# faris-k/self-supervised-wafermaps

Hardware: AMD Instinct MI355X
Metric: imgs/sec (SimCLR ResNet18, bs=256, 224^2) (higher is better)
Workload: dtype bf16; 1 GPU; SimCLR ResNet-18, 256 wafers/GPU/step, two 3x224x224 views, NT-Xent in-batch negatives, SGD (BASELINE.json configs[1]); per_gpu_batch=256, global_batch=256, parallelism=dp1, hip_graph=True, backward_stage_graphs=1, parallel_branches=two views through the backbone

## Files before the change

self-supervised-wafermaps_amd/csrc/bn.hip:

```cpp
#include "common.h"

namespace {

constexpr int BN_THREADS = 256;

__device__ __forceinline__ void unpack8(const uint4 v, float (&f)[8]) {
  f[0] = bf2f((uint16_t)(v.x & 0xffff)); f[1] = bf2f((uint16_t)(v.x >> 16));
  f[2] = bf2f((uint16_t)(v.y & 0xffff)); f[3] = bf2f((uint16_t)(v.y >> 16));
  f[4] = bf2f((uint16_t)(v.z & 0xffff)); f[5] = bf2f((uint16_t)(v.z >> 16));
  f[6] = bf2f((uint16_t)(v.w & 0xffff)); f[7] = bf2f((uint16_t)(v.w >> 16));
}
__device__ __forceinline__ uint4 pack8(const float (&f)[8]) {
  return make_uint4(pack_bf2(f[0], f[1]), pack_bf2(f[2], f[3]), pack_bf2(f[4], f[5]), pack_bf2(f[6], f[7]));
}

struct PoolSrc {
  const uint16_t* dy;
  const uint8_t* idx;
  int H, W, P, Q;
};

__device__ __forceinline__ void pool_grad8(const PoolSrc& ps, uint32_t row, int C, int c0, float (&g)[8]) {
  const uint32_t hw = (uint32_t)(ps.H * ps.W);
  const int n = (int)(row / hw);
// ... 373 lines not shown
        coef[((size_t)g * 7 + 1) * C + c] = is;
        coef[((size_t)g * 7 + 2) * C + c] = sc;
        coef[((size_t)g * 7 + 3) * C + c] = (float)(s1 / rows_per_group);
        coef[((size_t)g * 7 + 4) * C + c] = (float)(s2 / rows_per_group);
        coef[((size_t)g * 7 + 5) * C + c] = sc;
        coef[((size_t)g * 7 + 6) * C + c] = (beta ? beta[c] : 0.f) - mu * sc;
      }
    }
  }
  if (owner) {
    if (dgamma) dgamma[c] = (accumulate ? dgamma[c] : 0.f) + (float)tg;
    if (dbeta) dbeta[c] = (accumulate ? dbeta[c] : 0.f) + (float)tb;
  }
}

template <bool POW2, int FORM>
__global__ __launch_bounds__(BN_THREADS, FORM == 0 ? 4 : 1) void bn_bwd_apply(const uint16_t* __restrict__ y,
                                                           const uint16_t* __restrict__ dout,
                                                           const uint16_t* __restrict__ out,
                                                           const float* __restrict__ coef,
                                                           long long rows, int C, int rows_per_group,
                                                           int remask, int cshift, uint16_t* __restrict__ dy,
                                                           uint16_t* __restrict__ dz, const PoolSrc ps) {
  const int cpr = C >> 3;
  const long long total = rows * cpr;
  int cur_g = -1;
  constexpr int NK = FORM == 0 ? 5 : 7;
  float k[NK][8];
  for (long long p = (long long)blockIdx.x * BN_THREADS + threadIdx.x; p < total;
       p += (long long)gridDim.x * BN_THREADS) {
    long long row;
    int c0, g;
    if (POW2) {
      row = p >> cshift;
      c0 = (int)(p & (cpr - 1)) * 8;
      g = 0;
      for (long long lim = rows_per_group; row >= lim; lim += rows_per_group) ++g;
    } else {
      row = p / cpr;
      c0 = (int)(p - row * cpr) * 8;
      g = (int)(row / rows_per_group);
    }
    if (!POW2 || g != cur_g) {
      const float* cf = coef + (size_t)g * 7 * C + c0;
#pragma unroll
      for (int t = 0; t < NK; ++t) {
        const float4 a = *reinterpret_cast<const float4*>(cf + (size_t)t * C);
        const float4 b = *reinterpret_cast<const float4*>(cf + (size_t)t * C + 4);
        k[t][0] = a.x; k[t][1] = a.y; k[t][2] = a.z; k[t][3] = a.w;
        k[t][4] = b.x; k[t][5] = b.y; k[t][6] = b.z; k[t][7] = b.w;
      }
      cur_g = g;
    }
    const size_t off = row * C + c0;
    float fy[8], fd[8];
    unpack8(*reinterpret_cast<const uint4*>(y + off), fy);
    if constexpr (FORM == 2) pool_grad8(ps, (uint32_t)row, C, c0, fd);
    else unpack8(*reinterpret_cast<const uint4*>(dout + off), fd);
    if constexpr (FORM != 0) {
      if (out) {
        float fo[8];
        unpack8(*reinterpret_cast<const uint4*>(out + off), fo);
#pragma unroll
        for (int e = 0; e < 8; ++e) fd[e] = fo[e] > 0.f ? fd[e] : 0.f;
      }
      if (!out && remask) {
#pragma unroll
        for (int e = 0; e < 8; ++e) fd[e] = bf2f(f2bf(fmaf(fy[e], k[NK - 2][e], k[NK - 1][e]))) > 0.f ? fd[e] : 0.f;
      }
      if (dz) *reinterpret_cast<uint4*>(dz + off) = pack8(fd);
    }
    float r[8];
#pragma unroll
    for (int e = 0; e < 8; ++e) {
      const float xh = (fy[e] - k[0][e]) * k[1][e];
      r[e] = k[2][e] * (fd[e] - k[3][e] - xh * k[4][e]);
    }
    *reinterpret_cast<uint4*>(dy + off) = pack8(r);
  }
}

__global__ __launch_bounds__(BN_THREADS) void bn_pool_bwd_apply(const uint16_t* __restrict__ y,
                                                                const float* __restrict__ coef, int n_coef, int N, int C,
                                                                int imgs_per_group, int remask,
                                                                uint16_t* __restrict__ dy, const PoolSrc ps,
                                                                const WmDiv d_cpr, const WmDiv d_wb, const WmDiv d_ha,
                                                                const WmDiv d_ipg) {
  const uint32_t cpr = (uint32_t)C >> 3;
  const uint32_t HA = (uint32_t)ps.H >> 1, WB = (uint32_t)ps.W >> 1;
  const uint32_t total = (uint32_t)N * HA * WB * cpr;
  extern __shared__ __attribute__((aligned(16))) float pool_coef[];
  for (int i = threadIdx.x; i < n_coef; i += BN_THREADS) pool_coef[i] = coef[i];
  __syncthreads();
  for (uint32_t t = blockIdx.x * BN_THREADS + threadIdx.x; t < total; t += gridDim.x * BN_THREADS) {
    uint32_t rc, rb, ra;
    uint32_t u = wm_divmod(t, d_cpr, rc);
    const int c0 = (int)rc * 8;
    u = wm_divmod(u, d_wb, rb);
    const int n = (int)wm_divmod(u, d_ha, ra);
    const int b = (int)rb, a = (int)ra;
    const int g = (int)wm_div((uint32_t)n, d_ipg);
    const float* kk = pool_coef + (size_t)g * 7 * C + c0;
    auto krow = [&](int q, float (&v)[8]) {
      const float4 lo = *reinterpret_cast<const float4*>(kk + q * C);
      const float4 hi = *reinterpret_cast<const float4*>(kk + q * C + 4);
      v[0] = lo.x; v[1] = lo.y; v[2] = lo.z; v[3] = lo.w; v[4] = hi.x; v[5] = hi.y; v[6] = hi.z; v[7] = hi.w;
    };
    uint2 pk[4];
    uint4 dv[4];
    bool wok[4];
#pragma unroll
    for (int j = 0; j < 4; ++j) {
      const int p = a + (j >> 1), q = b + (j & 1);
      wok[j] = p < ps.P && q < ps.Q;
      const int pc = p < ps.P ? p : ps.P - 1, qc = q < ps.Q ? q : ps.Q - 1;
      const size_t o = ((size_t)(n * ps.P + pc) * ps.Q + qc) * C + c0;
      pk[j] = *reinterpret_cast<const uint2*>(ps.idx + o);
      dv[j] = *reinterpret_cast<const uint4*>(ps.dy + o);
    }
    float dw[4][8];
#pragma unroll
    for (int j = 0; j < 4; ++j) unpack8(dv[j], dw[j]);
#pragma unroll
    for (int pix = 0; pix < 4; ++pix) {
      const int dh = pix >> 1, dwp = pix & 1;
      float fd[8];
#pragma unroll
      for (int e = 0; e < 8; ++e) fd[e] = 0.f;
#pragma unroll
      for (int j = 0; j < 4; ++j) {
        const int kh = dh + 1 - 2 * (j >> 1), kw = dwp + 1 - 2 * (j & 1);
        if (kh < 0 || kw < 0) continue;
        const int code = kh * 3 + kw;
        if (wok[j]) {
#pragma unroll
          for (int e = 0; e < 8; ++e) {
            const int ie = (int)(((e < 4 ? pk[j].x : pk[j].y) >> (8 * (e & 3))) & 0xff);
            fd[e] += ie == code ? dw[j][e] : 0.f;
          }
        }
      }
#pragma unroll
      for (int e = 0; e < 8; ++e) fd[e] = bf2f(f2bf(fd[e]));
      const size_t off = ((size_t)(n * ps.H + 2 * a + dh) * ps.W + 2 * b + dwp) * C + c0;
      float fy[8];
      unpack8(*reinterpret_cast<const uint4*>(y + off), fy);
      if (remask) {
        float k5[8], k6[8];
        krow(5, k5);
        krow(6, k6);
#pragma unroll
        for (int e = 0; e < 8; ++e) fd[e] = bf2f(f2bf(fmaf(fy[e], k5[e], k6[e]))) > 0.f ? fd[e] : 0.f;
      }
      float r[8], k0[8], k1[8];
      krow(0, k0);
      krow(1, k1);
#pragma unroll
      for (int e = 0; e < 8; ++e) r[e] = (fy[e] - k0[e]) * k1[e];
      krow(4, k0);
      krow(3, k1);
#pragma unroll
      for (int e = 0; e < 8; ++e) r[e] = fd[e] - k1[e] - r[e] * k0[e];
      krow(2, k0);
#pragma unroll
      for (int e = 0; e < 8; ++e) r[e] = k0[e] * r[e];
      *reinterpret_cast<uint4*>(dy + off) = pack8(r);
    }
  }
}

__global__ __launch_bounds__(BN_THREADS) void stats_prereduce(const float* __restrict__ in, int T, int R, int To, int GC2,
                                                              int C2, float* __restrict__ out) {
  const long long i = (long long)blockIdx.x * BN_THREADS + threadIdx.x;
  const long long total = (long long)GC2 / C2 * To * C2;
  if (i >= total) return;
  const int c2 = (int)(i % C2);
  const long long u = i / C2;
  const int to = (int)(u % To), g = (int)(u / To);
  const float* src = in + ((size_t)g * T + (size_t)to * R) * C2 + c2;
  const int n = min(R, T - to * R);
  float v = 0.f;
  int k = 0;
  for (; k + 8 <= n; k += 8) {
    float t[8];
#pragma unroll
    for (int q = 0; q < 8; ++q) t[q] = src[(size_t)(k + q) * C2];
#pragma unroll
    for (int q = 0; q < 8; ++q) v += t[q];
  }
  for (; k < n; ++k) v += src[(size_t)k * C2];
  out[i] = v;
}

constexpr int STAT_SLOTS_DIRECT = 512, STAT_SLOTS_REDUCED = 128;
inline size_t stat_scratch_floats(int T, int G, int C) {
  return T > STAT_SLOTS_DIRECT ? (size_t)G * STAT_SLOTS_REDUCED * 2 * C : 0;
}

inline const float* stat_partials(const float* stat_part, int T, int G, int C, float* scratch, int* nblk, hipStream_t st) {
  if (T <= STAT_SLOTS_DIRECT) {
    *nblk = T;
    return stat_part;
  }
  int R = 1;
  while ((T + R - 1) / R > STAT_SLOTS_REDUCED) R *= 2;
  const int To = (T + R - 1) / R;
  const long long total = (long long)G * To * 2 * C;
  stats_prereduce<<<wm_cdiv(total, BN_THREADS), BN_THREADS, 0, st>>>(stat_part, T, R, To, G * 2 * C, 2 * C, scratch);
  *nblk = To;
  return scratch;
}

inline bool chunk_pow2(int C, int* shift) {
  const int cpr = C >> 3;
  if (cpr <= 0 || (cpr & (cpr - 1)) || BN_THREADS % cpr) return false;
  int sft = 0;
  while ((1 << sft) < cpr) ++sft;
  *shift = sft;
  return true;
}

__global__ __launch_bounds__(BN_THREADS) void add_bf16_kernel(const uint16_t* __restrict__ a,
                                                              const uint16_t* __restrict__ b,
                                                              long long n8, uint16_t* __restrict__ o) {
  for (long long p = (long long)blockIdx.x * BN_THREADS + threadIdx.x; p < n8;
       p += (long long)gridDim.x * BN_THREADS) {
    float fa[8], fb[8];
    unpack8(reinterpret_cast<const uint4*>(a)[p], fa);
    unpack8(reinterpret_cast<const uint4*>(b)[p], fb);
#pragma unroll
    for (int e = 0; e < 8; ++e) fa[e] += fb[e];
    reinterpret_cast<uint4*>(o)[p] = pack8(fa);
  }
}

inline int reduce_blocks(int rows_per_group, int C) {
  const int tpr = C >> 3;
  const int rpp = BN_THREADS / tpr > 0 ? BN_THREADS / tpr : 1;
  int nblk = wm_cdiv(rows_per_group, rpp * 16);
  if (nblk > 256) nblk = 256;
  if (nblk < 1) nblk = 1;
  return nblk;
}

inline int stream_grid(long long items) {
  long long b = (items + BN_THREADS - 1) / BN_THREADS;
  if (b > 256 * 16) b = 256 * 16;
  if (b < 1) b = 1;
  return (int)b;
// ... 206 lines not shown
  launch_finalize(bn_fwd_finalize, C, st, part, nblk, G, C, rpg, 0, gamma, beta, eps, momentum, running_mean, running_var,
                  num_batches_tracked, save_mean, save_invstd, scale, shift);
  WM_LAUNCH_CHECK();
  return WM_OK;
}

int bn_train_fwd_impl(const void* y_, const void* residual, const float* gamma, const float* beta, float* running_mean,
                      float* running_var, long long* num_batches_tracked, long long rows, int C, int G, float eps,
                      float momentum, int relu, float* save_mean, float* save_invstd, void* out_, void* relu_mask,
                      const float* stat_part, int stat_tiles, void* workspace, size_t workspace_bytes, void* stream) {
  WM_REQUIRE(y_ && out_ && save_mean && save_invstd && workspace, WM_EINVAL);
  const int rc = bn_shape_check(rows, C, G);
  if (rc != WM_OK) return rc;
  const size_t need = stat_part ? ((size_t)2 * G * C + stat_scratch_floats(stat_tiles, G, C)) * sizeof(float)
                                : wm_bn_workspace_bytes(rows, C, G);
  WM_REQUIRE(workspace_bytes >= need, WM_EWORKSPACE);
  hipStream_t st = static_cast<hipStream_t>(stream);
  const uint16_t *y = bf16(y_), *res = bf16(residual);
  uint16_t* out = bf16(out_);
  const int rpg = (int)(rows / G);
  if (!stat_part && bn_wide(rows, C, G)) {
    WM_REQUIRE(relu_mask == nullptr, WM_EUNSUPPORTED);
    bn_col_fwd<<<wm_cdiv(C, BN_THREADS), BN_THREADS, 0, st>>>(y, res, gamma, beta, running_mean, running_var,
                                                              num_batches_tracked, rpg, C, G, eps, momentum, relu, 1,
                                                              save_mean, save_invstd, out);
    WM_LAUNCH_CHECK();
    return WM_OK;
  }
  float* scale = static_cast<float*>(workspace);
  float* shift = scale + (size_t)G * C;
  const int rs = bn_fwd_stats(y, stat_part, stat_tiles, gamma, beta, running_mean, running_var, num_batches_tracked, rpg, C, G,
                              eps, momentum, save_mean, save_invstd, scale, shift, shift + (size_t)G * C, st);
  if (rs != WM_OK) return rs;
  launch_bn_apply(y, res, scale, shift, rows, C, rpg, relu, out, st, static_cast<uint8_t*>(relu_mask));
  WM_LAUNCH_CHECK();
  return WM_OK;
}

int bn_bwd_impl(const void* y_, const void* dout_, const void* out_relu_, int relu_from_y, const float* gamma,
                const float* beta, const float* save_mean, const float* save_invstd, long long rows, int C, int G,
                float* dgamma, float* dbeta, int accumulate, void* dy_, void* dz_, void* workspace, size_t workspace_bytes,
                void* stream, const PoolSrc ps, const void* ysel) {
  WM_REQUIRE(y_ && (dout_ || ps.dy) && save_mean && save_invstd && dy_ && workspace, WM_EINVAL);
  const int rc = bn_shape_check(rows, C, G);
  if (rc != WM_OK) return rc;
  WM_REQUIRE(workspace_bytes >= wm_bn_workspace_bytes(rows, C, G), WM_EWORKSPACE);
  hipStream_t st = static_cast<hipStream_t>(stream);
  const uint16_t *y = bf16(y_), *dout = bf16(dout_), *out_relu = bf16(out_relu_);
  uint16_t *dy = bf16(dy_), *dz = bf16(dz_);
  const int rpg = (int)(rows / G);
  const bool remask = relu_remask(relu_from_y, out_relu);
  if (bn_wide(rows, C, G)) {
    WM_REQUIRE(ps.dy == nullptr && dout, WM_EUNSUPPORTED);
    bn_col_bwd<<<wm_cdiv(C, BN_THREADS), BN_THREADS, 0, st>>>(y, dout, out_relu, remask ? 1 : 0, gamma, beta, save_mean,
                                                              save_invstd, rpg, C, G, dgamma, dbeta, accumulate, dy, dz);
    WM_LAUNCH_CHECK();
    return WM_OK;
  }
  const int nblk = reduce_blocks(rpg, C);
  float* part = static_cast<float*>(workspace);
  float* coef = part + (size_t)G * nblk * 2 * C;
  const int tpr = C >> 3;
  WM_REQUIRE(!remask || (gamma && beta), WM_EINVAL);
  int nblk_used = nblk;
  if (ps.dy != nullptr && ysel != nullptr) {
    const long long prow = (long long)(rows / ((long long)ps.H * ps.W)) * ps.P * ps.Q;
    WM_REQUIRE(prow % G == 0, WM_EUNSUPPORTED);
    const int prpg = (int)(prow / G);
    nblk_used = reduce_blocks(prpg, C);
    if (nblk_used > nblk) nblk_used = nblk;
    launch_reduce<1>(bf16(ysel), ps.dy, nullptr, save_mean, save_invstd, gamma, beta, prpg, C, G, nblk_used, part, PoolSrc{},
                     st);
  } else {
    launch_reduce<1>(y, dout, out_relu, save_mean, save_invstd, remask ? gamma : nullptr, remask ? beta : nullptr, rpg, C, G,
                     nblk, part, ps, st);
  }
  WM_LAUNCH_CHECK();
  launch_finalize(bn_bwd_finalize, C, st, part, nblk_used, G, C, rpg, gamma, beta, save_mean, save_invstd, dgamma, dbeta,
                  accumulate, coef, 0);
  WM_LAUNCH_CHECK();
  if (ps.dy != nullptr && !dz && !out_relu && (ps.H & 1) == 0 && (ps.W & 1) == 0 && BN_THREADS % tpr == 0 &&
      rows * tpr < (1ll << 31) && (size_t)G * 7 * C * sizeof(float) <= 32768) {
    const int n_img = (int)(rows / ((long long)ps.H * ps.W));
    bn_pool_bwd_apply<<<stream_grid(rows / 4 * tpr), BN_THREADS, (size_t)G * 7 * C * sizeof(float), st>>>(
        y, coef, G * 7 * C, n_img, C, n_img / G, remask ? 1 : 0, dy, ps, wm_div_make((uint32_t)(C >> 3)),
        wm_div_make((uint32_t)(ps.W >> 1)), wm_div_make((uint32_t)(ps.H >> 1)), wm_div_make((uint32_t)(n_img / G)));
    WM_LAUNCH_CHECK();
    return WM_OK;
  }
  const int form = ps.dy != nullptr ? 2 : (out_relu == nullptr && !remask && dz == nullptr) ? 0 : 1;
  launch_bn_bwd_apply(form, y, dout, out_relu, coef, rows, C, rpg, remask, dy, dz, ps, st);
  WM_LAUNCH_CHECK();
  return WM_OK;
}

}

extern "C" size_t wm_bn_workspace_bytes(long long rows, int C, int G) {
  if (rows <= 0 || C <= 0 || G <= 0 || C % 8) return 0;
  const int nblk = reduce_blocks((int)(rows / G), C);
  return ((size_t)G * nblk * 2 * C + (size_t)G * 7 * C) * sizeof(float) + 256;
}

extern "C" int wm_bn_train_fwd(const void* y, const void* residual, const float* gamma,
                               const float* beta, float* running_mean, float* running_var,
                               long long* num_batches_tracked, long long rows, int C, int G, float eps, float momentum, int relu,
                               float* save_mean, float* save_invstd, void* out, void* relu_mask, void* workspace,
                               size_t workspace_bytes, void* stream) {
  return bn_train_fwd_impl(y, residual, gamma, beta, running_mean, running_var, num_batches_tracked, rows, C, G, eps, momentum,
                           relu, save_mean, save_invstd, out, relu_mask, nullptr, 0, workspace, workspace_bytes, stream);
}

extern "C" int wm_bn_train_fwd_from_stats(const void* y, const void* residual, const float* gamma,
                                          const float* beta, float* running_mean, float* running_var,
                                          long long* num_batches_tracked, long long rows, int C, int G, float eps,
                                          float momentum, int relu,
                                          float* save_mean, float* save_invstd, void* out, void* relu_mask,
                                          const float* stat_part, int stat_tiles, void* workspace,
                                          size_t workspace_bytes, void* stream) {
  WM_REQUIRE(stat_part && stat_tiles > 0, WM_EINVAL);
  return bn_train_fwd_impl(y, residual, gamma, beta, running_mean, running_var, num_batches_tracked, rows, C, G, eps, momentum,
                           relu, save_mean, save_invstd, out, relu_mask, stat_part, stat_tiles, workspace, workspace_bytes,
                           stream);
}

extern "C" int wm_bn_train_stats(const void* y, const float* gamma, const float* beta, float* running_mean,
                                 float* running_var, long long* num_batches_tracked, long long rows, int C, int G, float eps, float momentum,
                                 float* save_mean, float* save_invstd, float* scale, float* shift, const float* stat_part,
                                 int stat_tiles, void* workspace, size_t workspace_bytes, void* stream) {
  WM_REQUIRE(y && save_mean && save_invstd && scale && shift && workspace, WM_EINVAL);
  const int rc = bn_shape_check(rows, C, G);
  if (rc != WM_OK) return rc;
  WM_REQUIRE(!stat_part || stat_tiles > 0, WM_EINVAL);
  WM_REQUIRE(workspace_bytes >= fwd_partials_bytes(stat_part, stat_tiles, rows, C, G), WM_EWORKSPACE);
  return bn_fwd_stats(bf16(y), stat_part, stat_tiles, gamma, beta, running_mean, running_var, num_batches_tracked,
                      (int)(rows / G), C, G, eps, momentum, save_mean, save_invstd, scale, shift,
                      static_cast<float*>(workspace), static_cast<hipStream_t>(stream));
}

extern "C" int wm_bn_eval_scale_shift(const float* gamma, const float* beta, const float* running_mean,
                                      const float* running_var, int C, float eps, float* scale, float* shift,
                                      void* stream) {
  WM_REQUIRE(running_mean && running_var && scale && shift && C > 0, WM_EINVAL);
  launch_eval_params(gamma, beta, running_mean, running_var, eps, C, scale, shift, static_cast<hipStream_t>(stream));
  WM_LAUNCH_CHECK();
  return WM_OK;
}

extern "C" int wm_bn_eval_fwd(const void* y_, const void* residual, const float* gamma, const float* beta,
                              const float* running_mean, const float* running_var, long long rows, int C,
                              float eps, int relu, void* out_, void* workspace, size_t workspace_bytes,
                              void* stream) {
  WM_REQUIRE(y_ && out_ && running_mean && running_var && workspace, WM_EINVAL);
  const int rc = bn_shape_check(rows, C, 1);
  if (rc != WM_OK) return rc;
  WM_REQUIRE(workspace_bytes >= (size_t)2 * C * sizeof(float), WM_EWORKSPACE);
  hipStream_t st = static_cast<hipStream_t>(stream);
  const uint16_t *y = bf16(y_), *res = bf16(residual);
  uint16_t* out = bf16(out_);
  if (bn_wide(rows, C, 1)) {
    bn_col_fwd<<<wm_cdiv(C, BN_THREADS), BN_THREADS, 0, st>>>(y, res, gamma, beta, const_cast<float*>(running_mean),
                                                              const_cast<float*>(running_var), nullptr, (int)rows, C, 1, eps,
                                                              0.f, relu, 0, nullptr, nullptr, out);
    WM_LAUNCH_CHECK();
    return WM_OK;
  }
  float* scale = static_cast<float*>(workspace);
  float* shift = scale + C;
  launch_eval_params(gamma, beta, running_mean, running_var, eps, C, scale, shift, st);
// ... 165 lines not shown
```

self-supervised-wafermaps_amd/csrc/pool.hip:

```cpp
#include "common.h"

namespace {

constexpr int PL_THREADS = 256;

__device__ __forceinline__ void up8(const uint4 v, float (&f)[8]) {
  f[0] = bf2f((uint16_t)(v.x & 0xffff)); f[1] = bf2f((uint16_t)(v.x >> 16));
  f[2] = bf2f((uint16_t)(v.y & 0xffff)); f[3] = bf2f((uint16_t)(v.y >> 16));
  f[4] = bf2f((uint16_t)(v.z & 0xffff)); f[5] = bf2f((uint16_t)(v.z >> 16));
  f[6] = bf2f((uint16_t)(v.w & 0xffff)); f[7] = bf2f((uint16_t)(v.w >> 16));
}

__global__ __launch_bounds__(PL_THREADS) void maxpool_fwd(const uint16_t* __restrict__ x, int N, int H,
                                                          int W, int C, int P, int Q,
                                                          uint16_t* __restrict__ y,
                                                          uint8_t* __restrict__ idx) {
  const int cpr = C >> 3;
  const long long total = (long long)N * P * Q * cpr;
  for (long long t = (long long)blockIdx.x * PL_THREADS + threadIdx.x; t < total;
       t += (long long)gridDim.x * PL_THREADS) {
    const int c0 = (int)(t % cpr) * 8;
    long long pix = t / cpr;
    const int q = (int)(pix % Q);
    pix /= Q;
    const int p = (int)(pix % P), n = (int)(pix / P);
    float best[8];
    int bi[8];
#pragma unroll
    for (int e = 0; e < 8; ++e) {
      best[e] = -INFINITY;
      bi[e] = 0;
    }
    bool first = true;
#pragma unroll
    for (int kh = 0; kh < 3; ++kh)
#pragma unroll
      for (int kw = 0; kw < 3; ++kw) {
        const int h = p * 2 - 1 + kh, w = q * 2 - 1 + kw;
        if ((unsigned)h < (unsigned)H && (unsigned)w < (unsigned)W) {
          float f[8];
          up8(*reinterpret_cast<const uint4*>(x + ((size_t)(n * H + h) * W + w) * C + c0), f);
#pragma unroll
          for (int e = 0; e < 8; ++e)
            if (first || f[e] > best[e]) {
              best[e] = f[e];
              bi[e] = kh * 3 + kw;
            }
          first = false;
        }
      }
    const size_t o = ((size_t)(n * P + p) * Q + q) * C + c0;
    *reinterpret_cast<uint4*>(y + o) = make_uint4(pack_bf2(best[0], best[1]), pack_bf2(best[2], best[3]),
                                                  pack_bf2(best[4], best[5]), pack_bf2(best[6], best[7]));
    uint2 pk;
    pk.x = bi[0] | (bi[1] << 8) | (bi[2] << 16) | (bi[3] << 24);
    pk.y = bi[4] | (bi[5] << 8) | (bi[6] << 16) | (bi[7] << 24);
    *reinterpret_cast<uint2*>(idx + o) = pk;
  }
}

__global__ __launch_bounds__(PL_THREADS) void bn_relu_maxpool_fwd(const uint16_t* __restrict__ x,
                                                                  const float* __restrict__ scale,
                                                                  const float* __restrict__ shift, int N,
                                                                  int H, int W, int C, int P, int Q,
                                                                  int imgs_per_group,
                                                                  uint16_t* __restrict__ y,
                                                                  uint8_t* __restrict__ idx,
                                                                  uint16_t* __restrict__ xsel, const WmDiv d_cpr,
                                                                  const WmDiv d_q, const WmDiv d_p, const WmDiv d_ipg) {
  const uint32_t cpr = (uint32_t)C >> 3;
  const uint32_t total = (uint32_t)N * P * Q * cpr;
  for (uint32_t t = blockIdx.x * PL_THREADS + threadIdx.x; t < total; t += gridDim.x * PL_THREADS) {
    uint32_t rc, rq, rp;
    uint32_t pix = wm_divmod(t, d_cpr, rc);
    const int c0 = (int)rc * 8;
    pix = wm_divmod(pix, d_q, rq);
    const int n = (int)wm_divmod(pix, d_p, rp);
    const int q = (int)rq, p = (int)rp;
    const int g = (int)wm_div((uint32_t)n, d_ipg);
    float sc[8], sh[8], bx[8];
#pragma unroll
    for (int e = 0; e < 8; ++e) {
      sc[e] = scale[(size_t)g * C + c0 + e];
      sh[e] = shift[(size_t)g * C + c0 + e];
    }
    float best[8];
    int bi[8];
#pragma unroll
    for (int e = 0; e < 8; ++e) {
      best[e] = -INFINITY;
      bi[e] = 0;
    }
    bool first = true;
#pragma unroll
    for (int kh = 0; kh < 3; ++kh)
#pragma unroll
      for (int kw = 0; kw < 3; ++kw) {
        const int h = p * 2 - 1 + kh, w = q * 2 - 1 + kw;
        if ((unsigned)h < (unsigned)H && (unsigned)w < (unsigned)W) {
          float f[8];
          up8(*reinterpret_cast<const uint4*>(x + ((size_t)(n * H + h) * W + w) * C + c0), f);
#pragma unroll
          for (int e = 0; e < 8; ++e) {
            const float v = bf2f(f2bf(fmaxf(fmaf(f[e], sc[e], sh[e]), 0.f)));
            if (first || v > best[e]) {
              best[e] = v;
              bi[e] = kh * 3 + kw;
              bx[e] = f[e];
            }
          }
          first = false;
        }
      }
    const size_t o = ((size_t)(n * P + p) * Q + q) * C + c0;
    *reinterpret_cast<uint4*>(y + o) = make_uint4(pack_bf2(best[0], best[1]), pack_bf2(best[2], best[3]),
                                                  pack_bf2(best[4], best[5]), pack_bf2(best[6], best[7]));
    uint2 pk;
    pk.x = bi[0] | (bi[1] << 8) | (bi[2] << 16) | (bi[3] << 24);
    pk.y = bi[4] | (bi[5] << 8) | (bi[6] << 16) | (bi[7] << 24);
    *reinterpret_cast<uint2*>(idx + o) = pk;
    if (xsel != nullptr)
      *reinterpret_cast<uint4*>(xsel + o) = make_uint4(pack_bf2(bx[0], bx[1]), pack_bf2(bx[2], bx[3]),
                                                       pack_bf2(bx[4], bx[5]), pack_bf2(bx[6], bx[7]));
  }
}

__global__ __launch_bounds__(PL_THREADS) void maxpool_bwd(const uint16_t* __restrict__ dy,
                                                          const uint8_t* __restrict__ idx, int N, int H,
                                                          int W, int C, int P, int Q,
                                                          uint16_t* __restrict__ dx) {
  const int cpr = C >> 3;
  const long long total = (long long)N * H * W * cpr;
  for (long long t = (long long)blockIdx.x * PL_THREADS + threadIdx.x; t < total;
       t += (long long)gridDim.x * PL_THREADS) {
    const int c0 = (int)(t % cpr) * 8;
    long long pix = t / cpr;
    const int w = (int)(pix % W);
    pix /= W;
    const int h = (int)(pix % H), n = (int)(pix / H);
    float g[8];
#pragma unroll
    for (int e = 0; e < 8; ++e) g[e] = 0.f;
    const int p_lo = h >> 1, p_hi = (h + 1) >> 1, q_lo = w >> 1, q_hi = (w + 1) >> 1;
    for (int p = p_lo; p <= p_hi; ++p) {
      if (p >= P) continue;
      const int kh = h - (2 * p - 1);
      for (int q = q_lo; q <= q_hi; ++q) {
        if (q >= Q) continue;
        const int code = kh * 3 + (w - (2 * q - 1));
        const size_t o = ((size_t)(n * P + p) * Q + q) * C + c0;
        const uint2 pk = *reinterpret_cast<const uint2*>(idx + o);
        float d[8];
        up8(*reinterpret_cast<const uint4*>(dy + o), d);
#pragma unroll
        for (int e = 0; e < 8; ++e) {
          const int ie = (int)(((e < 4 ? pk.x : pk.y) >> (8 * (e & 3))) & 0xff);
          g[e] += ie == code ? d[e] : 0.f;
        }
      }
    }
    *reinterpret_cast<uint4*>(dx + ((size_t)(n * H + h) * W + w) * C + c0) =
        make_uint4(pack_bf2(g[0], g[1]), pack_bf2(g[2], g[3]), pack_bf2(g[4], g[5]), pack_bf2(g[6], g[7]));
  }
}

__global__ __launch_bounds__(PL_THREADS) void gap_fwd(const uint16_t* __restrict__ x, int N, int HW, int C,
                                                      uint16_t* __restrict__ y) {
  const int cpr = C >> 3;
  const int t = blockIdx.x * PL_THREADS + threadIdx.x;
  if (t >= N * cpr) return;
  const int n = t / cpr, c0 = (t - n * cpr) * 8;
  float s[8];
#pragma unroll
  for (int e = 0; e < 8; ++e) s[e] = 0.f;
  for (int i = 0; i < HW; ++i) {
    float f[8];
    up8(*reinterpret_cast<const uint4*>(x + ((size_t)n * HW + i) * C + c0), f);
#pragma unroll
    for (int e = 0; e < 8; ++e) s[e] += f[e];
  }
  const float inv = 1.0f / (float)HW;
  *reinterpret_cast<uint4*>(y + (size_t)n * C + c0) =
      make_uint4(pack_bf2(s[0] * inv, s[1] * inv), pack_bf2(s[2] * inv, s[3] * inv),
                 pack_bf2(s[4] * inv, s[5] * inv), pack_bf2(s[6] * inv, s[7] * inv));
}

__global__ __launch_bounds__(PL_THREADS) void gap_bwd(const uint16_t* __restrict__ dy, int N, int HW, int C,
                                                      uint16_t* __restrict__ dx) {
  const int cpr = C >> 3;
  const long long total = (long long)N * HW * cpr;
  const float inv = 1.0f / (float)HW;
  for (long long t = (long long)blockIdx.x * PL_THREADS + threadIdx.x; t < total;
       t += (long long)gridDim.x * PL_THREADS) {
    const int c0 = (int)(t % cpr) * 8;
    const long long pix = t / cpr;
    const int n = (int)(pix / HW);
    float d[8];
    up8(*reinterpret_cast<const uint4*>(dy + (size_t)n * C + c0), d);
    *reinterpret_cast<uint4*>(dx + (size_t)pix * C + c0) =
        make_uint4(pack_bf2(d[0] * inv, d[1] * inv), pack_bf2(d[2] * inv, d[3] * inv),
                   pack_bf2(d[4] * inv, d[5] * inv), pack_bf2(d[6] * inv, d[7] * inv));
  }
}

inline int grid_for(long long items) {
  long long b = (items + PL_THREADS - 1) / PL_THREADS;
  if (b > 4096) b = 4096;
  return b < 1 ? 1 : (int)b;
}

}

extern "C" int wm_maxpool3x3s2_fwd(const void* x, int N, int H, int W, int C, void* y, void* idx, void* stream) {
  WM_REQUIRE(x && y && idx, WM_EINVAL);
  WM_REQUIRE(N > 0 && H > 1 && W > 1 && C > 0, WM_EINVAL);
  WM_REQUIRE(C % 8 == 0, WM_EUNSUPPORTED);
  const int P = (H + 2 - 3) / 2 + 1, Q = (W + 2 - 3) / 2 + 1;
  maxpool_fwd<<<grid_for((long long)N * P * Q * (C >> 3)), PL_THREADS, 0, static_cast<hipStream_t>(stream)>>>(
      static_cast<const uint16_t*>(x), N, H, W, C, P, Q, static_cast<uint16_t*>(y), static_cast<uint8_t*>(idx));
  WM_LAUNCH_CHECK();
  return WM_OK;
}

extern "C" int wm_bn_relu_maxpool3x3s2_fwd(const void* x, const float* scale, const float* shift, int N, int H,
                                           int W, int C, int G, void* y, void* idx, void* xsel, void* stream) {
  WM_REQUIRE(x && scale && shift && y && idx, WM_EINVAL);
  WM_REQUIRE(N > 0 && H > 1 && W > 1 && C > 0 && G > 0, WM_EINVAL);
  WM_REQUIRE(C % 8 == 0 && N % G == 0, WM_EUNSUPPORTED);
  WM_REQUIRE((long long)N * H * W * (C / 8) < (1ll << 31), WM_EUNSUPPORTED);
  const int P = (H + 2 - 3) / 2 + 1, Q = (W + 2 - 3) / 2 + 1;
  bn_relu_maxpool_fwd<<<grid_for((long long)N * P * Q * (C >> 3)), PL_THREADS, 0, static_cast<hipStream_t>(stream)>>>(
      static_cast<const uint16_t*>(x), scale, shift, N, H, W, C, P, Q, N / G, static_cast<uint16_t*>(y),
      static_cast<uint8_t*>(idx), static_cast<uint16_t*>(xsel), wm_div_make((uint32_t)(C >> 3)), wm_div_make((uint32_t)Q),
      wm_div_make((uint32_t)P), wm_div_make((uint32_t)(N / G)));
  WM_LAUNCH_CHECK();
  return WM_OK;
}

extern "C" int wm_maxpool3x3s2_bwd(const void* dy, const void* idx, int N, int H, int W, int C, void* dx,
                                   void* stream) {
  WM_REQUIRE(dy && idx && dx, WM_EINVAL);
  WM_REQUIRE(N > 0 && H > 1 && W > 1 && C > 0, WM_EINVAL);
  WM_REQUIRE(C % 8 == 0, WM_EUNSUPPORTED);
  const int P = (H + 2 - 3) / 2 + 1, Q = (W + 2 - 3) / 2 + 1;
  maxpool_bwd<<<grid_for((long long)N * H * W * (C >> 3)), PL_THREADS, 0, static_cast<hipStream_t>(stream)>>>(
      static_cast<const uint16_t*>(dy), static_cast<const uint8_t*>(idx), N, H, W, C, P, Q,
      static_cast<uint16_t*>(dx));
  WM_LAUNCH_CHECK();
  return WM_OK;
}

extern "C" int wm_gap_fwd(const void* x, int N, int HW, int C, void* y, void* stream) {
  WM_REQUIRE(x && y, WM_EINVAL);
  WM_REQUIRE(N > 0 && HW > 0 && C > 0, WM_EINVAL);
  WM_REQUIRE(C % 8 == 0, WM_EUNSUPPORTED);
  gap_fwd<<<wm_cdiv((long long)N * (C >> 3), PL_THREADS), PL_THREADS, 0, static_cast<hipStream_t>(stream)>>>(
      static_cast<const uint16_t*>(x), N, HW, C, static_cast<uint16_t*>(y));
  WM_LAUNCH_CHECK();
  return WM_OK;
}

extern "C" int wm_gap_bwd(const void* dy, int N, int HW, int C, void* dx, void* stream) {
  WM_REQUIRE(dy && dx, WM_EINVAL);
  WM_REQUIRE(N > 0 && HW > 0 && C > 0, WM_EINVAL);
  WM_REQUIRE(C % 8 == 0, WM_EUNSUPPORTED);
  gap_bwd<<<grid_for((long long)N * HW * (C >> 3)), PL_THREADS, 0, static_cast<hipStream_t>(stream)>>>(
      static_cast<const uint16_t*>(dy), N, HW, C, static_cast<uint16_t*>(dx));
  WM_LAUNCH_CHECK();
  return WM_OK;
}
```

Baseline: 24650 imgs/sec.

## Process two pool rows per thread in fused BN-ReLU-maxpool forward and backward

The fused BN+ReLU+maxpool forward now gives each thread two output rows. It loads a 5x3 input window once, so overlapping input rows are reused, and it picks the max with packed integer keys that encode the value and kernel position, removing the per-element branchy compare. The backward BN-pool apply kernel likewise handles two pooled rows per thread. It issues all dy/idx/y loads before the LDS coefficient staging barrier to hide latency, and switches from a grid-stride loop to an exact grid with XCD swizzle. This raises register pressure and makes index math 32-bit only, in exchange for fewer redundant loads and better memory-level parallelism.

```diff
diff --git a/self-supervised-wafermaps_amd/csrc/bn.hip b/self-supervised-wafermaps_amd/csrc/bn.hip
--- a/self-supervised-wafermaps_amd/csrc/bn.hip
+++ b/self-supervised-wafermaps_amd/csrc/bn.hip
@@ -479,45 +479,70 @@
 
 __global__ __launch_bounds__(BN_THREADS) void bn_pool_bwd_apply(const uint16_t* __restrict__ y,
                                                                 const float* __restrict__ coef, int n_coef, int N, int C,
-                                                                int imgs_per_group, int remask,
-                                                                uint16_t* __restrict__ dy, const PoolSrc ps,
-                                                                const WmDiv d_cpr, const WmDiv d_wb, const WmDiv d_ha,
+                                                                int remask, uint16_t* __restrict__ dy, const PoolSrc ps,
+                                                                const WmDiv d_cpr, const WmDiv d_wb, const WmDiv d_ha2,
                                                                 const WmDiv d_ipg) {
   const uint32_t cpr = (uint32_t)C >> 3;
   const uint32_t HA = (uint32_t)ps.H >> 1, WB = (uint32_t)ps.W >> 1;
-  const uint32_t total = (uint32_t)N * HA * WB * cpr;
+  const uint32_t total = (uint32_t)N * d_ha2.d * WB * cpr;
   extern __shared__ __attribute__((aligned(16))) float pool_coef[];
-  for (int i = threadIdx.x; i < n_coef; i += BN_THREADS) pool_coef[i] = coef[i];
-  __syncthreads();
-  for (uint32_t t = blockIdx.x * BN_THREADS + threadIdx.x; t < total; t += gridDim.x * BN_THREADS) {
-    uint32_t rc, rb, ra;
-    uint32_t u = wm_divmod(t, d_cpr, rc);
-    const int c0 = (int)rc * 8;
-    u = wm_divmod(u, d_wb, rb);
-    const int n = (int)wm_divmod(u, d_ha, ra);
-    const int b = (int)rb, a = (int)ra;
-    const int g = (int)wm_div((uint32_t)n, d_ipg);
-    const float* kk = pool_coef + (size_t)g * 7 * C + c0;
-    auto krow = [&](int q, float (&v)[8]) {
-      const float4 lo = *reinterpret_cast<const float4*>(kk + q * C);
-      const float4 hi = *reinterpret_cast<const float4*>(kk + q * C + 4);
-      v[0] = lo.x; v[1] = lo.y; v[2] = lo.z; v[3] = lo.w; v[4] = hi.x; v[5] = hi.y; v[6] = hi.z; v[7] = hi.w;
-    };
-    uint2 pk[4];
-    uint4 dv[4];
-    bool wok[4];
-#pragma unroll
-    for (int j = 0; j < 4; ++j) {
-      const int p = a + (j >> 1), q = b + (j & 1);
-      wok[j] = p < ps.P && q < ps.Q;
-      const int pc = p < ps.P ? p : ps.P - 1, qc = q < ps.Q ? q : ps.Q - 1;
-      const size_t o = ((size_t)(n * ps.P + pc) * ps.Q + qc) * C + c0;
-      pk[j] = *reinterpret_cast<const uint2*>(ps.idx + o);
-      dv[j] = *reinterpret_cast<const uint4*>(ps.dy + o);
-    }
-    float dw[4][8];
-#pragma unroll
-    for (int j = 0; j < 4; ++j) unpack8(dv[j], dw[j]);
+  const int n_coef4 = n_coef >> 2;
+  const float4* coef4 = reinterpret_cast<const float4*>(coef);
+  float4 coef_first = make_float4(0.f, 0.f, 0.f, 0.f);
+  if ((int)threadIdx.x < n_coef4) coef_first = coef4[threadIdx.x];
+  const uint32_t t_raw = wm_xcd_swizzle(blockIdx.x, gridDim.x) * BN_THREADS + threadIdx.x;
+  const bool active = t_raw < total;
+  const uint32_t t = active ? t_raw : total - 1;
+  uint32_t rc, rb, rk;
+  uint32_t u = wm_divmod(t, d_cpr, rc);
+  const int c0 = (int)rc * 8;
+  u = wm_divmod(u, d_wb, rb);
+  const uint32_t n = wm_divmod(u, d_ha2, rk);
+  const int b = (int)rb, a0 = 2 * (int)rk;
+  const int g = (int)wm_div(n, d_ipg);
+  const float* kk = pool_coef + (size_t)g * 7 * C + c0;
+  auto krow = [&](int q, float (&v)[8]) {
+    const float4 lo = *reinterpret_cast<const float4*>(kk + q * C);
+    const float4 hi = *reinterpret_cast<const float4*>(kk + q * C + 4);
+    v[0] = lo.x; v[1] = lo.y; v[2] = lo.z; v[3] = lo.w; v[4] = hi.x; v[5] = hi.y; v[6] = hi.z; v[7] = hi.w;
+  };
+  const uint2* idx2 = reinterpret_cast<const uint2*>(ps.idx);
+  const uint4* pdy4 = reinterpret_cast<const uint4*>(ps.dy);
+  uint2 pk[6];
+  uint4 dv[6];
+  bool wok[6];
+#pragma unroll
+  for (int j = 0; j < 6; ++j) {
+    const int p = a0 + (j >> 1), q = b + (j & 1);
+    wok[j] = p < ps.P && q < ps.Q;
+    const int pc = p < ps.P ? p : ps.P - 1, qc = q < ps.Q ? q : ps.Q - 1;
+    const uint32_t o = ((n * (uint32_t)ps.P + (uint32_t)pc) * (uint32_t)ps.Q + (uint32_t)qc) * cpr + rc;
+    pk[j] = idx2[o];
+    dv[j] = pdy4[o];
+  }
+  const uint4* y4 = reinterpret_cast<const uint4*>(y);
+  uint4 yv[8];
+#pragma unroll
+  for (int i = 0; i < 8; ++i) {
+    const int a = a0 + (i >> 2), dh = (i >> 1) & 1, dwp = i & 1;
+    const int ac = (uint32_t)a < HA ? a : a0;
+    yv[i] = y4[((n * (uint32_t)ps.H + (uint32_t)(2 * ac + dh)) * (uint32_t)ps.W + (uint32_t)(2 * b + dwp)) * cpr + rc];
+  }
+  {
+    float4* lds4 = reinterpret_cast<float4*>(pool_coef);
+    if ((int)threadIdx.x < n_coef4) lds4[threadIdx.x] = coef_first;
+    for (int i = threadIdx.x + BN_THREADS; i < n_coef4; i += BN_THREADS) lds4[i] = coef4[i];
+    __syncthreads();
+  }
+  if (!active) return;
+  float dw[6][8];
+#pragma unroll
+  for (int j = 0; j < 6; ++j) unpack8(dv[j], dw[j]);
+  uint4* dy4 = reinterpret_cast<uint4*>(dy);
+#pragma unroll
+  for (int s = 0; s < 2; ++s) {
+    const int a = a0 + s;
+    if (s == 1 && (uint32_t)a >= HA) break;
 #pragma unroll
     for (int pix = 0; pix < 4; ++pix) {
       const int dh = pix >> 1, dwp = pix & 1;
@@ -529,19 +554,20 @@
         const int kh = dh + 1 - 2 * (j >> 1), kw = dwp + 1 - 2 * (j & 1);
         if (kh < 0 || kw < 0) continue;
         const int code = kh * 3 + kw;
-        if (wok[j]) {
+        const int jw = j + 2 * s;
+        if (wok[jw]) {
 #pragma unroll
           for (int e = 0; e < 8; ++e) {
-            const int ie = (int)(((e < 4 ? pk[j].x : pk[j].y) >> (8 * (e & 3))) & 0xff);
-            fd[e] += ie == code ? dw[j][e] : 0.f;
+            const int ie = (int)(((e < 4 ? pk[jw].x : pk[jw].y) >> (8 * (e & 3))) & 0xff);
+            fd[e] += ie == code ? dw[jw][e] : 0.f;
           }
         }
       }
 #pragma unroll
       for (int e = 0; e < 8; ++e) fd[e] = bf2f(f2bf(fd[e]));
-      const size_t off = ((size_t)(n * ps.H + 2 * a + dh) * ps.W + 2 * b + dwp) * C + c0;
+      const uint32_t off = ((n * (uint32_t)ps.H + (uint32_t)(2 * a + dh)) * (uint32_t)ps.W + (uint32_t)(2 * b + dwp)) * cpr + rc;
       float fy[8];
-      unpack8(*reinterpret_cast<const uint4*>(y + off), fy);
+      unpack8(yv[4 * s + pix], fy);
       if (remask) {
         float k5[8], k6[8];
         krow(5, k5);
@@ -561,7 +587,7 @@
       krow(2, k0);
 #pragma unroll
       for (int e = 0; e < 8; ++e) r[e] = k0[e] * r[e];
-      *reinterpret_cast<uint4*>(dy + off) = pack8(r);
+      dy4[off] = pack8(r);
     }
   }
 }
@@ -934,9 +960,11 @@
   if (ps.dy != nullptr && !dz && !out_relu && (ps.H & 1) == 0 && (ps.W & 1) == 0 && BN_THREADS % tpr == 0 &&
       rows * tpr < (1ll << 31) && (size_t)G * 7 * C * sizeof(float) <= 32768) {
     const int n_img = (int)(rows / ((long long)ps.H * ps.W));
-    bn_pool_bwd_apply<<<stream_grid(rows / 4 * tpr), BN_THREADS, (size_t)G * 7 * C * sizeof(float), st>>>(
-        y, coef, G * 7 * C, n_img, C, n_img / G, remask ? 1 : 0, dy, ps, wm_div_make((uint32_t)(C >> 3)),
-        wm_div_make((uint32_t)(ps.W >> 1)), wm_div_make((uint32_t)(ps.H >> 1)), wm_div_make((uint32_t)(n_img / G)));
+    const int ha2 = ((ps.H >> 1) + 1) / 2;
+    bn_pool_bwd_apply<<<wm_cdiv((long long)n_img * ha2 * (ps.W >> 1) * tpr, BN_THREADS), BN_THREADS,
+                        (size_t)G * 7 * C * sizeof(float), st>>>(
+        y, coef, G * 7 * C, n_img, C, remask ? 1 : 0, dy, ps, wm_div_make((uint32_t)(C >> 3)),
+        wm_div_make((uint32_t)(ps.W >> 1)), wm_div_make((uint32_t)ha2), wm_div_make((uint32_t)(n_img / G)));
     WM_LAUNCH_CHECK();
     return WM_OK;
   }
diff --git a/self-supervised-wafermaps_amd/csrc/pool.hip b/self-supervised-wafermaps_amd/csrc/pool.hip
--- a/self-supervised-wafermaps_amd/csrc/pool.hip
+++ b/self-supervised-wafermaps_amd/csrc/pool.hip
@@ -3,6 +3,7 @@
 namespace {
 
 constexpr int PL_THREADS = 256;
+typedef short s16x2_t __attribute__((ext_vector_type(2)));
 
 __device__ __forceinline__ void up8(const uint4 v, float (&f)[8]) {
   f[0] = bf2f((uint16_t)(v.x & 0xffff)); f[1] = bf2f((uint16_t)(v.x >> 16));
@@ -59,69 +60,121 @@
   }
 }
 
-__global__ __launch_bounds__(PL_THREADS) void bn_relu_maxpool_fwd(const uint16_t* __restrict__ x,
-                                                                  const float* __restrict__ scale,
-                                                                  const float* __restrict__ shift, int N,
-                                                                  int H, int W, int C, int P, int Q,
-                                                                  int imgs_per_group,
-                                                                  uint16_t* __restrict__ y,
-                                                                  uint8_t* __restrict__ idx,
-                                                                  uint16_t* __restrict__ xsel, const WmDiv d_cpr,
-                                                                  const WmDiv d_q, const WmDiv d_p, const WmDiv d_ipg) {
+template <bool XSEL>
+__global__ __launch_bounds__(PL_THREADS, 4) void bn_relu_maxpool_fwd(const uint16_t* __restrict__ x,
+                                                                     const float* __restrict__ scale,
+                                                                     const float* __restrict__ shift, int N,
+                                                                     int H, int W, int C, int P, int Q,
+                                                                     uint16_t* __restrict__ y,
+                                                                     uint8_t* __restrict__ idx,
+                                                                     uint16_t* __restrict__ xsel, const WmDiv d_cpr,
+                                                                     const WmDiv d_q, const WmDiv d_p2, const WmDiv d_ipg) {
   const uint32_t cpr = (uint32_t)C >> 3;
-  const uint32_t total = (uint32_t)N * P * Q * cpr;
-  for (uint32_t t = blockIdx.x * PL_THREADS + threadIdx.x; t < total; t += gridDim.x * PL_THREADS) {
-    uint32_t rc, rq, rp;
-    uint32_t pix = wm_divmod(t, d_cpr, rc);
-    const int c0 = (int)rc * 8;
-    pix = wm_divmod(pix, d_q, rq);
-    const int n = (int)wm_divmod(pix, d_p, rp);
-    const int q = (int)rq, p = (int)rp;
-    const int g = (int)wm_div((uint32_t)n, d_ipg);
-    float sc[8], sh[8], bx[8];
-#pragma unroll
-    for (int e = 0; e < 8; ++e) {
-      sc[e] = scale[(size_t)g * C + c0 + e];
-      sh[e] = shift[(size_t)g * C + c0 + e];
-    }
-    float best[8];
-    int bi[8];
-#pragma unroll
-    for (int e = 0; e < 8; ++e) {
-      best[e] = -INFINITY;
-      bi[e] = 0;
-    }
-    bool first = true;
-#pragma unroll
-    for (int kh = 0; kh < 3; ++kh)
-#pragma unroll
-      for (int kw = 0; kw < 3; ++kw) {
-        const int h = p * 2 - 1 + kh, w = q * 2 - 1 + kw;
-        if ((unsigned)h < (unsigned)H && (unsigned)w < (unsigned)W) {
-          float f[8];
-          up8(*reinterpret_cast<const uint4*>(x + ((size_t)(n * H + h) * W + w) * C + c0), f);
-#pragma unroll
-          for (int e = 0; e < 8; ++e) {
-            const float v = bf2f(f2bf(fmaxf(fmaf(f[e], sc[e], sh[e]), 0.f)));
-            if (first || v > best[e]) {
-              best[e] = v;
-              bi[e] = kh * 3 + kw;
-              bx[e] = f[e];
-            }
+  const uint32_t total = (uint32_t)N * d_p2.d * (uint32_t)Q * cpr;
+  const uint32_t t = wm_xcd_swizzle(blockIdx.x, gridDim.x) * PL_THREADS + threadIdx.x;
+  if (t >= total) return;
+  uint32_t rc, rq, rj;
+  uint32_t pix = wm_divmod(t, d_cpr, rc);
+  pix = wm_divmod(pix, d_q, rq);
+  const uint32_t n = wm_divmod(pix, d_p2, rj);
+  const uint32_t g = wm_div(n, d_ipg);
+  const int q = (int)rq, p0 = 2 * (int)rj;
+  float sc[8], sh[8];
+  {
+    const float* ps = scale + (size_t)g * C + rc * 8;
+    const float* ph = shift + (size_t)g * C + rc * 8;
+    const float4 sa = *reinterpret_cast<const float4*>(ps), sb = *reinterpret_cast<const float4*>(ps + 4);
+    const float4 ha = *reinterpret_cast<const float4*>(ph), hb = *reinterpret_cast<const float4*>(ph + 4);
+    sc[0] = sa.x; sc[1] = sa.y; sc[2] = sa.z; sc[3] = sa.w; sc[4] = sb.x; sc[5] = sb.y; sc[6] = sb.z; sc[7] = sb.w;
+    sh[0] = ha.x; sh[1] = ha.y; sh[2] = ha.z; sh[3] = ha.w; sh[4] = hb.x; sh[5] = hb.y; sh[6] = hb.z; sh[7] = hb.w;
+  }
+  const uint4* x4 = reinterpret_cast<const uint4*>(x);
+  const int h0 = 2 * p0 - 1, w0 = 2 * q - 1;
+  uint32_t colc[3], kwpart[3];
+#pragma unroll
+  for (int kw = 0; kw < 3; ++kw) {
+    const int w = w0 + kw;
+    colc[kw] = (uint32_t)(w < 0 ? 0 : w >= W ? W - 1 : w) * cpr;
+    kwpart[kw] = (unsigned)w < (unsigned)W ? (uint32_t)(3 - kw) : 0u;
+  }
+  uint4 v[5][3];
+#pragma unroll
+  for (int r = 0; r < 5; ++r) {
+    const int h = h0 + r;
+    const uint32_t rowc = ((n * (uint32_t)H + (uint32_t)(h < 0 ? 0 : h >= H ? H - 1 : h)) * (uint32_t)W) * cpr + rc;
+#pragma unroll
+    for (int kw = 0; kw < 3; ++kw) v[r][kw] = x4[rowc + colc[kw]];
+  }
+  auto row_best = [&](const uint4 (&rv)[3], uint32_t (&rk)[8], float (&rx)[8]) {
+#pragma unroll
+    for (int kw = 0; kw < 3; ++kw) {
+      float f[8];
+      up8(rv[kw], f);
+#pragma unroll
+      for (int e = 0; e < 8; e += 2) {
+        const s16x2_t pat = __builtin_bit_cast(s16x2_t, pack_bf2(fmaf(f[e], sc[e], sh[e]), fmaf(f[e + 1], sc[e + 1], sh[e + 1])));
+        const uint32_t pk = __builtin_bit_cast(uint32_t, __builtin_elementwise_max(pat, s16x2_t{0, 0}));
+        const uint32_t key[2] = {(pk << 16) | kwpart[kw], (pk & 0xffff0000u) | kwpart[kw]};
+#pragma unroll
+        for (int u = 0; u < 2; ++u) {
+          if (kw == 0) {
+            rk[e + u] = key[u];
+            rx[e + u] = f[e + u];
+          } else {
+            const bool take = key[u] > rk[e + u];
+            rk[e + u] = take ? key[u] : rk[e + u];
+            rx[e + u] = take ? f[e + u] : rx[e + u];
           }
-          first = false;
         }
       }
-    const size_t o = ((size_t)(n * P + p) * Q + q) * C + c0;
-    *reinterpret_cast<uint4*>(y + o) = make_uint4(pack_bf2(best[0], best[1]), pack_bf2(best[2], best[3]),
-                                                  pack_bf2(best[4], best[5]), pack_bf2(best[6], best[7]));
+    }
+  };
+  auto merge = [&](uint32_t (&bk)[8], float (&bx)[8], const uint32_t (&rk)[8], const float (&rx)[8], uint32_t khpart) {
+#pragma unroll
+    for (int e = 0; e < 8; ++e) {
+      const uint32_t c = rk[e] + khpart;
+      const bool take = c > bk[e];
+      bk[e] = take ? c : bk[e];
+      bx[e] = take ? rx[e] : bx[e];
+    }
+  };
+  auto emit = [&](const uint32_t (&bk)[8], const float (&bx)[8], uint32_t pp) {
+    const uint32_t o = ((n * (uint32_t)P + pp) * (uint32_t)Q + (uint32_t)q) * cpr + rc;
+    reinterpret_cast<uint4*>(y)[o] =
+        make_uint4((bk[0] >> 16) | (bk[1] & 0xffff0000u), (bk[2] >> 16) | (bk[3] & 0xffff0000u),
+                   (bk[4] >> 16) | (bk[5] & 0xffff0000u), (bk[6] >> 16) | (bk[7] & 0xffff0000u));
+    uint32_t code[8];
+#pragma unroll
+    for (int e = 0; e < 8; ++e) code[e] = 9u - (bk[e] & 0xfu);
     uint2 pk;
-    pk.x = bi[0] | (bi[1] << 8) | (bi[2] << 16) | (bi[3] << 24);
-    pk.y = bi[4] | (bi[5] << 8) | (bi[6] << 16) | (bi[7] << 24);
-    *reinterpret_cast<uint2*>(idx + o) = pk;
-    if (xsel != nullptr)
-      *reinterpret_cast<uint4*>(xsel + o) = make_uint4(pack_bf2(bx[0], bx[1]), pack_bf2(bx[2], bx[3]),
-                                                       pack_bf2(bx[4], bx[5]), pack_bf2(bx[6], bx[7]));
+    pk.x = code[0] | (code[1] << 8) | (code[2] << 16) | (code[3] << 24);
+    pk.y = code[4] | (code[5] << 8) | (code[6] << 16) | (code[7] << 24);
+    reinterpret_cast<uint2*>(idx)[o] = pk;
+    if constexpr (XSEL)
+      reinterpret_cast<uint4*>(xsel)[o] = make_uint4(pack_bf2(bx[0], bx[1]), pack_bf2(bx[2], bx[3]),
+                                                     pack_bf2(bx[4], bx[5]), pack_bf2(bx[6], bx[7]));
+  };
+  uint32_t bk[8], rk[8], sk[8];
+  float bx[8], rx[8], sx[8];
+  row_best(v[0], bk, bx);
+  {
+    const uint32_t khpart0 = p0 > 0 ? 6u : 0u;
+#pragma unroll
+    for (int e = 0; e < 8; ++e) bk[e] += khpart0;
+  }
+  row_best(v[1], rk, rx);
+  merge(bk, bx, rk, rx, 3u);
+  row_best(v[2], sk, sx);
+  merge(bk, bx, sk, sx, 0u);
+  emit(bk, bx, (uint32_t)p0);
+  if (p0 + 1 < P) {
+#pragma unroll
+    for (int e = 0; e < 8; ++e) sk[e] += 6u;
+    row_best(v[3], rk, rx);
+    merge(sk, sx, rk, rx, 3u);
+    row_best(v[4], rk, rx);
+    merge(sk, sx, rk, rx, 0u);
+    emit(sk, sx, (uint32_t)p0 + 1u);
   }
 }
 
@@ -229,10 +282,11 @@
   WM_REQUIRE(C % 8 == 0 && N % G == 0, WM_EUNSUPPORTED);
   WM_REQUIRE((long long)N * H * W * (C / 8) < (1ll << 31), WM_EUNSUPPORTED);
   const int P = (H + 2 - 3) / 2 + 1, Q = (W + 2 - 3) / 2 + 1;
-  bn_relu_maxpool_fwd<<<grid_for((long long)N * P * Q * (C >> 3)), PL_THREADS, 0, static_cast<hipStream_t>(stream)>>>(
-      static_cast<const uint16_t*>(x), scale, shift, N, H, W, C, P, Q, N / G, static_cast<uint16_t*>(y),
+  const int P2 = (P + 1) / 2;
+  (xsel ? bn_relu_maxpool_fwd<true> : bn_relu_maxpool_fwd<false>)<<<wm_cdiv((long long)N * P2 * Q * (C >> 3), PL_THREADS), PL_THREADS, 0, static_cast<hipStream_t>(stream)>>>(
+      static_cast<const uint16_t*>(x), scale, shift, N, H, W, C, P, Q, static_cast<uint16_t*>(y),
       static_cast<uint8_t*>(idx), static_cast<uint16_t*>(xsel), wm_div_make((uint32_t)(C >> 3)), wm_div_make((uint32_t)Q),
-      wm_div_make((uint32_t)P), wm_div_make((uint32_t)(N / G)));
+      wm_div_make((uint32_t)P2), wm_div_make((uint32_t)(N / G)));
   WM_LAUNCH_CHECK();
   return WM_OK;
 }
```

After: 25080 imgs/sec, median of 6. 1.8% higher.
